# Kkuntal990/video-to-video-diffusion

Measured on AMD Instinct MI355X. Metric: ddim_steps_per_sec, higher is better.
Workload: dtype bf16; 1 GPU; DDIM-50 step (U-Net eval + update) on latent [1, 8, 48, 128, 128] = 8->48 slices @512x512, effective 264.66M U-Net (128x(1,2,4,4), latent 8), one volume per GPU, hipGraph-captured step; volumes_per_gpu=1, parallelism=dp1, full=False, finite_outputs=True

## Files before the change

include/ctsi.h:

```cpp
#ifndef CTSI_H
#define CTSI_H

#include <stddef.h>
#include <stdint.h>

#ifdef __cplusplus
extern "C" {
#endif

#define CTSI_OK 0
#define CTSI_ERR_INVALID (-1)
#define CTSI_ERR_UNSUPPORTED (-2)
#define CTSI_ERR_HIP (-3)

int ctsi_version(void);
int ctsi_ablation_build(void);
const char* ctsi_last_error(void);
int ctsi_device_available(void);

int ctsi_ncdhw_f32_to_ndhwc_bf16(const float* src, void* dst, int n, int c, int d, int h, int w,
                                 int c_total, int c_off, void* stream);
int ctsi_ndhwc_bf16_to_ncdhw_f32(const void* src, float* dst, int n, int c, int d, int h, int w,
                                 void* stream);
int ctsi_ncdhw_f32_to_ndhwc_f32(const float* src, float* dst, int n, int c, int d, int h, int w,
// ... 38 lines not shown
int ctsi_conv_plan_set_stream_tail(ctsi_conv_plan* plan, int on);
void ctsi_conv_plan_destroy(ctsi_conv_plan* plan);
int ctsi_conv_plan_out_dims(const ctsi_conv_plan* plan, int* d_out, int* h_out, int* w_out);
size_t ctsi_conv_plan_weight_bytes(const ctsi_conv_plan* plan);
int ctsi_conv_plan_tiles(const ctsi_conv_plan* plan);
int ctsi_conv_plan_tiles_per_sample(const ctsi_conv_plan* plan);
int ctsi_conv_plan_cout_pad(const ctsi_conv_plan* plan);
size_t ctsi_conv_plan_workspace_bytes(const ctsi_conv_plan* plan);
double ctsi_conv_plan_flops(const ctsi_conv_plan* plan);
int ctsi_conv_plan_config(const ctsi_conv_plan* plan, int* bm, int* bn, int* mode);
int ctsi_conv_plan_form(const ctsi_conv_plan* plan, int out[8]);
#define CTSI_PACK_GATHER 1
#define CTSI_PACK_GATHER_SMALL 2
#define CTSI_PACK_HALO 3
#define CTSI_PACK_K32 4
#define CTSI_PACK_HEAD 5
#define CTSI_PACK_STREAM_TAIL 6
#define CTSI_PACK_STEM 7
int ctsi_conv_plan_pack_layout(const ctsi_conv_plan* plan);
int ctsi_conv_plan_pack_weights(const ctsi_conv_plan* plan, const float* w_f32, void* packed,
                                void* stream);
int ctsi_conv_fwd(const ctsi_conv_plan* plan, const void* x1, const void* x2, const void* packed_w,
                  const float* bias, const ctsi_conv_out* out, void* stream);

int ctsi_gn_colsum(const void* x_bf16, float* colsum, int n, int c, int d, int h, int w,
                   int* tiles_per_sample, void* stream);
int ctsi_gn_colsum_tiles(int d, int h, int w);
int ctsi_gn_finalize(const float* colsum, double* sums, int n, int c, int c_pad, int groups,
                     int tiles_per_sample, int nclass, int accumulate, void* stream);
int ctsi_gn_apply(const void* x_bf16, void* y_bf16, const double* sums, const float* gamma,
                  const float* beta, int n, int c, int d, int h, int w, int d_stat, int groups, float eps,
                  int silu_pre, const float* tbias, int tbias_stride, const int* step_ptr,
                  const void* residual_bf16, int silu_post, void* stream);

int ctsi_attn_pv_supported(int c, int groups);
int ctsi_attn_pv(const float* depthsum, const double* sums, const float* gamma, const float* beta, const void* w_bf16,
                 const float* bias, void* out, int n, int c, int d, int h, int w, int groups, float eps, void* stream);

int ctsi_attn_depthsum(const void* x_bf16, float* depthsum, float* colsum, int n, int c, int d,
                       int h, int w, void* stream);
int ctsi_attn_depthsum_tiles(int c, int h, int w);
int ctsi_attn_normsum(const float* depthsum, const double* sums, const float* gamma,
                      const float* beta, void* out_bf16, int n, int c, int d, int h, int w,
                      int groups, float eps, void* stream);
int ctsi_attn_broadcast_add(const void* x_bf16, const void* p_bf16, const float* rowsum, int heads,
                            void* y_bf16, int n, int c, int d, int h, int w, void* stream);
int ctsi_attn_softmax_rowsum(const void* qk_bf16, float* rowsum, int n, int c, int d, int h, int w,
                             int heads, void* stream);

int ctsi_time_embed_fwd(const int* t_rows, int rows, int dim, int time_dim, const float* w1,
                        const float* b1, const float* w2, const float* b2, const float* w_all,
                        const float* b_all, int total_out, float* scratch, float* tbias_out,
                        void* stream);

int ctsi_time_embed_fwd_tf(const float* t_rows, int rows, int dim, int time_dim, const float* w1,
                           const float* b1, const float* w2, const float* b2, const float* w_all,
                           const float* b_all, int total_out, float* scratch, float* tbias_out,
                           void* stream);

int ctsi_trilinear_depth_fwd(const float* src_f32_ncdhw, void* dst_bf16_ndhwc, int n, int c,
                             int d_in, int d_out, int h, int w, int c_total, int c_off,
                             float* dst_f32_ncdhw, void* stream);

int ctsi_ddim_step(float* z, const float* eps, const float* noise_ncdhw, void* zin_bf16,
                   int c_total, int c_off, const float* coef, const int* step_ptr, int n, int c,
                   int d, int h, int w, int* nonfinite, void* stream);
// ... 174 lines not shown
```

video-to-video-diffusion_amd/csrc/norm_act.hip:

```cpp
#include "ctsi_internal.h"
#include <stdlib.h>

#define GN_TILE_ROWS 512

__device__ __forceinline__ void unpack8(const uint4 v, float* f) {
    f[0] = __uint_as_float(v.x << 16); f[1] = __uint_as_float(v.x & 0xffff0000u);
    f[2] = __uint_as_float(v.y << 16); f[3] = __uint_as_float(v.y & 0xffff0000u);
    f[4] = __uint_as_float(v.z << 16); f[5] = __uint_as_float(v.z & 0xffff0000u);
    f[6] = __uint_as_float(v.w << 16); f[7] = __uint_as_float(v.w & 0xffff0000u);
}
__device__ __forceinline__ uint4 pack8(const float* f) {
    uint4 v;
    v.x = pack_bf16x2(f[0], f[1]); v.y = pack_bf16x2(f[2], f[3]);
    v.z = pack_bf16x2(f[4], f[5]); v.w = pack_bf16x2(f[6], f[7]);
    return v;
}

__global__ void __launch_bounds__(256)
gn_colsum_kernel(const bf16_t* __restrict__ x, float* __restrict__ colsum, int n_total, int c,
                 long long vox_per_sample, int tps) {
    extern __shared__ __attribute__((aligned(16))) char smem_raw[];
    float* s_red = reinterpret_cast<float*>(smem_raw);
    const int cpr = c >> 3;
    const int rows_par = 256 / cpr;
// ... 329 lines not shown
    CTSI_CHECK_ARG(x && y && sums && gamma && beta, "ctsi_gn_apply: null argument");
    CTSI_CHECK_ARG(c % 8 == 0 && groups > 0 && c % groups == 0, "ctsi_gn_apply: bad c=%d groups=%d", c, groups);
    CTSI_CHECK_ARG(d_stat >= d, "ctsi_gn_apply: d_stat=%d < d=%d", d_stat, d);
    const long long vox = (long long)d * h * w;
    const long long total = vox * (c / 8);
    long long blocks = (total + 256 * 8 - 1) / (256 * 8);
    if (blocks > 2048) blocks = 2048;
    if (blocks < 1) blocks = 1;
    const int cpr = c / 8;
    int gq = cpr, g256 = 256;
    while (g256) { const int t = gq % g256; gq = g256; g256 = t; }
    const int need = cpr / gq;
    if (blocks >= need) blocks -= blocks % need;
    bool constq = (blocks * 256) % cpr == 0;
    long long per_block = 0;
    {
        static const char* cg = getenv("CTSI_GN_CONTIG");
        if (!(cg && atoi(cg) == 0) && 256 % cpr == 0) {
            per_block = 1024;
            blocks = (total + per_block - 1) / per_block;
            constq = true;
        }
    }
    const size_t lds = (size_t)c * 3 * sizeof(float);
    static const char* nt_env = getenv("CTSI_GN_NT");
    const bool nt = nt_env ? atoi(nt_env) != 0 : (long long)n * vox * c * 2 > (512ll << 20);
    const int idx = (silu_pre ? 1 : 0) | (tbias ? 2 : 0) | (residual ? 4 : 0) | (silu_post ? 8 : 0) | (constq ? 16 : 0) | (nt ? 32 : 0);
    hipLaunchKernelGGL(gn_apply_pick<0>(idx), dim3((unsigned)blocks, n), dim3(256), lds, (hipStream_t)stream,
                       (const bf16_t*)x, (bf16_t*)y, sums, gamma, beta, c, vox, (long long)d_stat * h * w, groups, eps,
                       tbias, tbias_stride, step_ptr, n, (const bf16_t*)residual, per_block);
    CTSI_LAUNCH_CHECK();
    return CTSI_OK;
}
```

video-to-video-diffusion_amd/engine.py:

```python
from __future__ import annotations

import contextlib
import ctypes as C
import os
import weakref
from typing import Callable, Dict, List, NamedTuple, Optional, Sequence, Tuple

import torch
import torch.nn as nn

from .lib import ConvDesc, ConvOut, CtsiError, get_lib
from .prediction import add_pred_to_eps, check_prediction_type

_CTX: Dict[int, "Ctx"] = {}

_PACKED: Dict[int, "weakref.WeakValueDictionary"] = {}
_LIVE_PROGRAMS: "weakref.WeakSet" = weakref.WeakSet()


def _pack_sig(lib, plan, transposed, k, s, c1: int, c2: int, cout: int, cin_w: Optional[int]) -> tuple:
    bm, bn, mode = C.c_int(), C.c_int(), C.c_int()
    lib.conv_plan_config(plan, C.byref(bm), C.byref(bn), C.byref(mode))
    return (lib.conv_plan_pack_layout(plan), int(transposed), tuple(k), tuple(s), c1, c2, cout, cin_w,
            lib.conv_plan_cout_pad(plan), lib.conv_plan_weight_bytes(plan), bn.value, bm.value,
# ... 631 lines not shown
    def gn_finalize(self, x: Act, groups: int, stats: dict) -> int:
        slot = self._gn_slot(x.n, groups)
        lib, sptr, prog = self.lib, self.ctx.sptr, self
        n, c = x.n, x.c
        parts = stats.get("parts") or [dict(tps=stats["tps"], cpad=stats["cpad"], nclass=stats["nclass"], off=0)]

        def run():
            for i, pt in enumerate(parts):
                lib.gn_finalize(C.c_void_p(prog._colsum.data_ptr() + pt["off"] * 4),
                                C.c_void_p(prog._gn_sums.data_ptr() + slot * 8), n, c, pt["cpad"], groups, pt["tps"],
                                pt["nclass"], int(i > 0), sptr)

        self._emit(run, "gn.finalize", audit=dict(kind="gn_finalize", colsum=lambda: prog._colsum, sums=lambda: prog._gn_sums,
                                                  slot=slot, n=n, c=c, groups=groups, parts=parts))
        return slot

    def gn_colsum(self, x: Act) -> dict:
        lib, sptr, prog = self.lib, self.ctx.sptr, self
        tps = lib.gn_colsum_tiles(x.d, x.h, x.w)
        self._colsum_need = max(self._colsum_need, 2 * x.n * tps * x.c)
        xp = x.ip
        n, c, d, h, w = x.n, x.c, x.d, x.h, x.w

        def run():
            lib.gn_colsum(xp, _ptr(prog._colsum), n, c, d, h, w, None, sptr)

        self._emit(run, "gn.colsum", nbytes=2.0 * n * c * d * h * w,
                   audit=dict(kind="gn_colsum", x=x, colsum=lambda: prog._colsum, tps=tps, tile_rows=512))
        return dict(tps=tps, cpad=x.c, nclass=1)

    def gn_apply(self, x: Act, slot: int, gn: nn.GroupNorm, *, silu_pre: bool, tbias=None,
                 tbias_off: int = 0, tbias_stride: int = 0, step_ptr: Optional[torch.Tensor] = None,
                 residual: Optional[Act] = None, silu_post: bool = False, out: Optional[Act] = None,
                 synced: bool = False) -> Act:
        lib, sptr, prog = self.lib, self.ctx.sptr, self
        if self.shard is not None and not synced:
            self.sync_stats_and_halos(x if x.halo else None, slot, x.n * gn.num_groups * 2)
        if residual is not None and self.shard is not None and residual.halo:
            self.halo_exchange(residual)
        lo, d_ext = self.ext(x)
        gamma = self.dev_f32(lambda: gn.weight)
        beta = self.dev_f32(lambda: gn.bias)
        self.track(gn.weight, gn.bias)
        fresh = out is None
        if out is None:
            out = self.act(x.n, x.c, x.d, x.h, x.w, halo=x.halo)
        out.dirty = bool(self.shard is not None and x.halo and x.dirty)
        xp, yp, gp, bp = self.ext_ptr(x, lo), self.ext_ptr(out, lo), _ptr(gamma), _ptr(beta)
        tbp = C.c_void_p(0 if tbias is None else tbias.data_ptr() + tbias_off * 4)
        stp = _ptr(step_ptr)
        rp = C.c_void_p(0) if residual is None else self.ext_ptr(residual, lo)
        n, c, h, w, groups, eps = x.n, x.c, x.h, x.w, gn.num_groups, float(gn.eps)
        d_stat = self.shard.depth_total if (self.shard is not None and x.halo) else x.d
        d = d_ext

        def run():
            lib.gn_apply(xp, yp, C.c_void_p(prog._gn_sums.data_ptr() + slot * 8), gp, bp, n, c, d, h, w, d_stat,
                         groups, eps, int(silu_pre), tbp, tbias_stride, stp, rp, int(silu_post), sptr)

        self._emit(run, "gn.apply", nbytes=(2 + (residual is not None)) * 2.0 * n * c * d * h * w,
                   audit=dict(kind="gn_apply", x=x, out=out, sums=lambda: prog._gn_sums, slot=slot, gamma=gamma, beta=beta,
                              groups=groups, eps=eps, d_stat=d_stat, silu_pre=bool(silu_pre), tbias=tbias, tbias_off=tbias_off,
                              tbias_stride=tbias_stride, step_ptr=step_ptr, residual=residual, silu_post=bool(silu_post)))
        if fresh:
            self.zero_end_halos(out)
        return out

    def unet_resblock(self, m, x: Act, skip: Optional[Act], tbias: torch.Tensor, tbias_off: int,
                      tbias_stride: int, step_ptr: Optional[torch.Tensor]) -> Act:
        cout = m.conv1.conv.out_channels
        has_res_conv = not isinstance(m.residual_conv, nn.Identity)
        if not has_res_conv and skip is not None:
            raise CtsiError("identity residual with a concatenated input")
        c1, st = self.conv("rb.conv1", lambda: m.conv1.conv.weight, lambda: m.conv1.conv.bias, x, skip,
                           cout=cout, want_stats=True)
        slot = self.gn_finalize(c1, m.conv1.norm.num_groups, st)
        c2, st = self.conv("rb.conv2", lambda: m.conv2[0].weight, lambda: m.conv2[0].bias, c1, None, cout=cout,
                           want_stats=True,
                           norm_in=(slot, m.conv1.norm, True, (tbias, tbias_off, tbias_stride, step_ptr)))
        self.release(c1)
        slot = self.gn_finalize(c2, m.conv2[1].num_groups, st)
        if not has_res_conv:
            return self.gn_apply(c2, slot, m.conv2[1], silu_pre=False, residual=x, silu_post=True, out=c2)
        if os.environ.get("CTSI_NO_FUSE_RES"):
            if self.shard is not None:
                for a in (x, skip):
                    if a is not None:
                        self.halo_exchange(a)
            r, _ = self.conv("res1x1", lambda: m.residual_conv.weight, lambda: m.residual_conv.bias, x, skip,
                             k=(1, 1, 1), p=(0, 0, 0), cout=cout, ext_out=self.shard is not None)
            out = self.gn_apply(c2, slot, m.conv2[1], silu_pre=False, residual=r, silu_post=True, out=c2)
            self.release(r)
            return out
        if self.shard is not None:
            self.sync_stats_and_halos(c2, slot, c2.n * m.conv2[1].num_groups * 2)
            for a in (x, skip):
                if a is not None:
                    self.halo_exchange(a)
        out, _ = self.conv("res1x1+gn", lambda: m.residual_conv.weight, lambda: m.residual_conv.bias, x, skip,
                           k=(1, 1, 1), p=(0, 0, 0), cout=cout, out=c2, fuse_gn=(c2, slot, m.conv2[1], True),
                           ext_out=self.shard is not None)
        return out

    def attention(self, m, x: Act, mode: str = "fast") -> Act:
        lib, sptr, prog = self.lib, self.ctx.sptr, self
        n, c, d, h, w = x.n, x.c, x.d, x.h, x.w
        dev = self.ctx.device
        heads = m.num_heads
        tps = lib.attn_depthsum_tiles(c, h, w)
        self._colsum_need = max(self._colsum_need, 2 * n * tps * c)
        depthsum = self.pool.get(n * h * w * c, torch.float32)
        xp, dsp = x.ip, _ptr(depthsum)
        world = self.shard.world if (self.shard is not None and x.halo) else 1
        d_all = self.shard.depth_total if (self.shard is not None and x.halo) else d

        def run_ds():
            lib.attn_depthsum(xp, dsp, _ptr(prog._colsum), n, c, d, h, w, sptr)

        self._emit(run_ds, "attn.depthsum", nbytes=2.0 * n * c * d * h * w,
                   audit=dict(kind="attn_depthsum", x=x, depthsum=depthsum, colsum=lambda: prog._colsum, tps=tps,
                              tile_pos=256 // (c // 8)))
        slot = self.gn_finalize(x, m.norm.num_groups, dict(tps=tps, cpad=c, nclass=1))
        if self.shard is not None and x.halo:
            self.sync_stats_and_halos(None, slot, n * m.norm.num_groups * 2, f32=depthsum, name="attn.sync")
            self.halo_exchange(x)
        gamma = self.dev_f32(lambda: m.norm.weight)
        beta = self.dev_f32(lambda: m.norm.bias)
        groups, eps = m.norm.num_groups, float(m.norm.eps)
        gp, bp = _ptr(gamma), _ptr(beta)

        def wv():
            return m.qkv.weight[2 * c:3 * c, :, 0, 0, 0].double()

        def wpv():
            wp = m.proj_out.weight[:, :, 0, 0, 0].double()
            return (wp @ wv()).float().reshape(c, c, 1, 1, 1)

        def bpv():
            wp = m.proj_out.weight[:, :, 0, 0, 0].double()
            return (float(d_all) * (wp @ m.qkv.bias[2 * c:3 * c].double()) + m.proj_out.bias.double()).float()

        if lib.attn_pv_supported(c, groups) and not os.environ.get("CTSI_NO_ATTN_PV"):
            wbuf = self.persistent((c, c), torch.bfloat16)
            self.pack_fns.append(lambda: wbuf.copy_(wpv().reshape(c, c).to(device=dev, dtype=torch.bfloat16)))
            bias_pv = self.dev_f32(bpv)
            pterm = self.act(n, c, 1, h, w, halo=0)
            wp_, bpp, ptp = _ptr(wbuf), _ptr(bias_pv), _ptr(pterm.t)

            def run_pv():
                lib.attn_pv(dsp, C.c_void_p(prog._gn_sums.data_ptr() + slot * 8), gp, bp, wp_, bpp, ptp, n, c, d_all, h, w,
                            groups, eps, sptr)

            fl_pv = 2.0 * n * h * w * c * c
            self.flops += fl_pv
# ... 113 lines not shown
                self.lib.graph_destroy(self._fast["graph"])
        except Exception:
            pass


class SamplerStep(NamedTuple):
    entry: str
    noise: bool
    hist: bool
    nonfinite: bool


SAMPLER_STEPS = {
    "ddim": SamplerStep("ddim_step", noise=True, hist=False, nonfinite=True),
    "ddpm": SamplerStep("ddpm_step", noise=True, hist=False, nonfinite=False),
    "dpmpp": SamplerStep("dpm_step", noise=False, hist=True, nonfinite=True),
    "heun": SamplerStep("heun_step", noise=True, hist=True, nonfinite=True),
}


def sampler_step_launcher(lib, kind: str, f32: bool) -> Callable:
    s = SAMPLER_STEPS[kind]
    fn = getattr(lib, s.entry + ("_f32" if f32 else ""))

    def launch(z, eps, hist, noise, zin, c_total, coef, step_ptr, n, L, d, h, w, nonfinite, stream):
        ops = [z, eps] + ([hist] if s.hist else []) + ([noise] if s.noise else [])
        tail = [nonfinite] if s.nonfinite else []
        fn(*ops, zin, c_total, 0, coef, step_ptr, n, L, d, h, w, *tail, stream)
    return launch


class UNetProgram(Program):

    def __init__(self, ctx: Ctx, unet, n: int, d: int, h: int, w: int, max_rows: int, attention_mode="fast",
                 shard=None, guided: bool = False, rescale: bool = False, prediction: str = "epsilon"):
        super().__init__(ctx)
        self.shard = shard
        if shard is not None and n != 1:
            raise CtsiError("depth-sharded programs support one volume per rank")
        if shard is not None and guided:
            raise CtsiError("classifier-free guidance does not support depth sharding: the sharded program holds one "
                            "volume per rank and the rescale statistics would need a collective")
        self.unet = unet
        self.guided, self.rescale = bool(guided), bool(guided and rescale)
        self.prediction = check_prediction_type(prediction)
        self.n, self.d, self.h, self.w = n, d, h, w
        n = self.nb = 2 * n if guided else n
        L = unet.latent_dim
        self.L = L
        dev = ctx.device
        self.attention_mode = attention_mode
        self.max_rows = max_rows
        halo = 0 if shard is None else 1
        self.xin, self.xin2 = self._input_acts(n, d, h, w, halo)
        self.eps = self.persistent((n, d, h, w, L), torch.float32)
        self.z = self.persistent((self.n, d, h, w, L), torch.float32, zero=True)
        self.step_ptr = self.persistent((1,), torch.int32, zero=True)
        self.t_rows = self.persistent((max_rows,), torch.int32, zero=True)
        self.t_rows_f = self.persistent((max_rows,), torch.float32, zero=True)
        self.coef = self.persistent((max_rows, 8), torch.float32, zero=True)
        self.noise = None
        self.track_module(unet)

        te = unet.time_embed.time_mlp
        self.dim = unet.model_channels
        self.time_dim = te[1].out_features
        blocks = [m for m in unet.modules() if type(m).__name__ == "ResBlock3D"]
        self.tb_off = {}
        off = 0
        for m in blocks:
            self.tb_off[id(m)] = off
            off += m.time_mlp[1].out_features
        self.total_out = off
        self.w1 = self.dev_f32(lambda: te[1].weight)
        self.b1 = self.dev_f32(lambda: te[1].bias)
        self.w2 = self.dev_f32(lambda: te[3].weight)
        self.b2 = self.dev_f32(lambda: te[3].bias)
        self.w_all = self.dev_f32(lambda: torch.cat([m.time_mlp[1].weight for m in blocks], 0))
        self.b_all = self.dev_f32(lambda: torch.cat([m.time_mlp[1].bias for m in blocks], 0))
        self.tbias = self.persistent((max_rows, self.total_out), torch.float32, zero=True)
        self.te_scratch = self.persistent((max_rows * (self.dim + 2 * self.time_dim),), torch.float32)

        self.zero_gn_op()
        x, _ = self.conv("conv_in", lambda: unet.conv_in.weight, lambda: unet.conv_in.bias, self.xin, self.xin2,
                         cout=unet.conv_in.out_channels)
        skips: List[Act] = []

        def step(layer, xcur: Act, skip: Optional[Act] = None) -> Act:
            ynew = self._layer(layer, xcur, skip)
            if not any(xcur is sk for sk in skips):
                self.release(xcur)
            if skip is not None:
                self.release(skip)
            return ynew

        for level_blocks, down in zip(unet.down_blocks, unet.down_samples):
            for block_list in level_blocks:
                for layer in block_list:
                    x = step(layer, x)
            skips.append(x)
            if not isinstance(down, nn.Identity):
                x, _ = self.conv("down", (lambda m=down: m.conv.weight), (lambda m=down: m.conv.bias), x, None,
                                 k=(3, 4, 4), s=(2, 2), p=(1, 1, 1), cout=down.conv.out_channels)
        x = step(unet.mid_block1, x)
        x = step(unet.mid_attn, x)
        x = step(unet.mid_block2, x)
        for level_blocks, up in zip(unet.up_blocks, unet.up_samples):
            for j, block_list in enumerate(level_blocks):
                skip = skips.pop() if j == 0 else None
                for layer in block_list:
                    x = step(layer, x, skip)
                    skip = None
            if not isinstance(up, nn.Identity):
                xo, _ = self.conv("up", (lambda m=up: m.conv.weight), (lambda m=up: m.conv.bias), x, None,
                                  transposed=True, k=(3, 4, 4), s=(2, 2), p=(1, 1, 1),
                                  cout=up.conv.out_channels)
                self.release(x)
                x = xo
        gn, conv = unet.conv_out[0], unet.conv_out[2]
        st = self.gn_colsum(x)
        slot = self.gn_finalize(x, gn.num_groups, st)
        y = self.gn_apply(x, slot, gn, silu_pre=True)
        self.release(x)
        vox = d * h * w
        self.conv("conv_out", lambda: conv.weight, lambda: conv.bias, y, None, cout=L, f32_out=self.eps,
                  f32_strides=(vox * L, 1, h * w * L, w * L, L))
        self.release(y)
        self.unet_op_count = len(self.ops)
        self.finalize_layout()

    def _input_acts(self, n, d, h, w, halo) -> Tuple[Act, Optional[Act]]:
        L = self.L
        return Act(self.persistent((n * (d + 2 * halo) * h * w * 2 * L,), torch.bfloat16, zero=True), n, 2 * L, d, h, w,
                   halo), None

    def _layer(self, layer, x: Act, skip: Optional[Act]) -> Act:
        kind = type(layer).__name__
        if kind == "ResBlock3D":
            return self.unet_resblock(layer, x, skip, self.tbias, self.tb_off[id(layer)], self.total_out,
                                      self.step_ptr)
        if kind == "TemporalAttention":
            return self.attention(layer, x, self.attention_mode)
        raise CtsiError(f"unsupported U-Net layer {kind}")

    def load_latents(self, z_ncdhw: Optional[torch.Tensor], cond_ncdhw: Optional[torch.Tensor]):
        lib, sptr = self.lib, self.ctx.sptr
        n, L, d, h, w = self.n, self.L, self.d, self.h, self.w
        lo = 0 if self.shard is None else self.shard.depth_start
        if z_ncdhw is not None:
            z = z_ncdhw.detach()[:, :, lo:lo + d].to(device=self.ctx.device, dtype=torch.float32).contiguous()
            lib.ncdhw_f32_to_ndhwc_f32(_ptr(z), _ptr(self.z), n, L, d, h, w, sptr)
            lib.ncdhw_f32_to_ndhwc_bf16(_ptr(z), self.xin.ip, n, L, d, h, w, 2 * L, 0, sptr)
            if self.guided:
                lib.ncdhw_f32_to_ndhwc_bf16(_ptr(z), self._uncond_zin(), n, L, d, h, w, 2 * L, 0, sptr)
            z.record_stream(self.ctx.stream)
            self.xin.dirty = True
        if cond_ncdhw is not None:
            cnd = cond_ncdhw.detach()[:, :, lo:lo + d].to(device=self.ctx.device, dtype=torch.float32).contiguous()
            lib.ncdhw_f32_to_ndhwc_bf16(_ptr(cnd), self.xin.ip, n, L, d, h, w, 2 * L, L, sptr)
            cnd.record_stream(self.ctx.stream)

    def set_guidance(self, scale: float, rescale: float = 0.0):
        if not self.guided:
            raise CtsiError("internal: set_guidance on a program built without guidance")
        if rescale > 0.0 and not self.rescale:
            raise CtsiError("internal: guidance_rescale > 0 needs a program built with the statistics pass")
        row = torch.tensor([float(scale), float(rescale)], dtype=torch.float32)
        self.cfg_scale.copy_(row.expand(self.cfg_scale.shape[0], 2))

    def set_schedule(self, t_rows: Sequence[float], coef_rows: Optional[torch.Tensor] = None,
                     pred_rows: Optional[torch.Tensor] = None):
        rows = len(t_rows)
        if rows > self.max_rows:
            raise CtsiError(f"schedule needs {rows} rows but the program was built for {self.max_rows}")
        lib, sptr = self.lib, self.ctx.sptr
# ... 312 lines not shown
```

video-to-video-diffusion_amd/engine_f32.py:

```python
from __future__ import annotations

import ctypes as C
import weakref
from typing import List, Optional, Tuple

import torch
import torch.nn as nn

from .engine import (_PACKED, Act, Ctx, UNetProgram, VAEDecodeProgram, VAEEncodeProgram, _content_key,
                     _ptr)
from .lib import ConvDesc, ConvOut, CtsiError

PRECISIONS = ("bf16", "fp32")


def _f32_pack_sig(desc: ConvDesc, cout_pad: int, wbytes: int) -> tuple:
    return ("fp32", int(desc.transposed), (desc.kd, desc.kh, desc.kw), (desc.sh, desc.sw), desc.c1, desc.c2, desc.cout,
            cout_pad, wbytes)


def check_precision(p) -> str:
    if not isinstance(p, str) or p not in PRECISIONS:
        raise ValueError(f"unknown inference precision {p!r}: expected one of {PRECISIONS}")
    return p


class _F32Ops:

    precision = "fp32"

    def act(self, n, c, d, h, w, halo: Optional[int] = None) -> Act:
        if halo:
            raise CtsiError("the fp32 inference mode does not support depth sharding")
        return Act(self.pool.get(n * c * d * h * w, torch.float32), n, c, d, h, w, 0)

    def conv(self, name: str, weight_fn, bias_fn, x1: Act, x2: Optional[Act], *, transposed=False, k=(3, 3, 3), s=(1, 1),
             p=(1, 1, 1), cout: int, cin_w: Optional[int] = None, out: Optional[Act] = None, want_stats=False,
             f32_out: Optional[torch.Tensor] = None, f32_strides=None, act: int = 0, fuse_gn=None, ext_out: bool = False,
             norm_in=None, residual: Optional[Act] = None):
        lib, prog = self.lib, self
        if fuse_gn is not None or ext_out:
            raise CtsiError("internal: the fused GroupNorm tail / halo-extended outputs are bf16-path features")
        c2 = 0 if x2 is None else x2.c
        if cin_w is not None and cin_w != x1.c + c2:
            raise CtsiError(f"internal: fp32 activations carry no padding channels (cin_w={cin_w}, c={x1.c + c2})")
        if x2 is not None and (x2.n, x2.d, x2.h, x2.w) != (x1.n, x1.d, x1.h, x1.w):
            raise CtsiError("internal: concatenated sources of different shapes")
        if norm_in is not None:
            nslot, ngn, nsilu, ntb = norm_in
            kw_tb = {} if ntb is None else dict(tbias=ntb[0], tbias_off=ntb[1], tbias_stride=ntb[2], step_ptr=ntb[3])
            self.gn_apply(x1, nslot, ngn, silu_pre=nsilu, out=x1, **kw_tb)
        desc = ConvDesc(int(transposed), k[0], k[1], k[2], s[0], s[1], p[0], p[1], p[2], x1.n, x1.c, c2, cout, x1.d, x1.h,
                        x1.w, 0)
        if not lib.conv_f32_supported(C.byref(desc)):
            raise CtsiError(f"{name}: {lib.last_error().decode()}")
        self.keep.append(desc)
        do, ho, wo, tps, ncls, cpad = (C.c_int() for _ in range(6))
        lib.conv_f32_geometry(C.byref(desc), C.byref(do), C.byref(ho), C.byref(wo), C.byref(tps), C.byref(ncls),
                              C.byref(cpad))
        do, ho, wo, tps, ncls, cpad = do.value, ho.value, wo.value, tps.value, ncls.value, cpad.value
# ... 241 lines not shown
```

video-to-video-diffusion_amd/lib.py:

```python
from __future__ import annotations

import ctypes as C
import os
import subprocess
from pathlib import Path

_PKG_DIR = Path(__file__).resolve().parent
LIB_PATH = _PKG_DIR / "libctsi.so"
CSRC_DIR = _PKG_DIR / "csrc"
HEADER_PATH = _PKG_DIR.parent / "include" / "ctsi.h"


class CtsiError(RuntimeError):
    """Raised when libctsi is unavailable or one of its entry points reports an error."""


class ConvDesc(C.Structure):
    _fields_ = [
        ("transposed", C.c_int),
        ("kd", C.c_int), ("kh", C.c_int), ("kw", C.c_int),
        ("sh", C.c_int), ("sw", C.c_int),
        ("pd", C.c_int), ("ph", C.c_int), ("pw", C.c_int),
        ("n", C.c_int), ("c1", C.c_int), ("c2", C.c_int),
        ("cout", C.c_int),
# ... 34 lines not shown
_vp, _i, _f, _ll, _sz = C.c_void_p, C.c_int, C.c_float, C.c_longlong, C.c_size_t
_ip = C.POINTER(C.c_int)

SIGNATURES = {
    "ctsi_version": (_i, [], False),
    "ctsi_ablation_build": (_i, [], False),
    "ctsi_last_error": (C.c_char_p, [], False),
    "ctsi_device_available": (_i, [], False),
    "ctsi_ncdhw_f32_to_ndhwc_bf16": (_i, [_vp, _vp, _i, _i, _i, _i, _i, _i, _i, _vp], True),
    "ctsi_ndhwc_bf16_to_ncdhw_f32": (_i, [_vp, _vp, _i, _i, _i, _i, _i, _vp], True),
    "ctsi_ncdhw_f32_to_ndhwc_f32": (_i, [_vp, _vp, _i, _i, _i, _i, _i, _vp], True),
    "ctsi_ndhwc_f32_to_ncdhw_f32": (_i, [_vp, _vp, _i, _i, _i, _i, _i, _vp], True),
    "ctsi_conv_plan_create": (_i, [C.POINTER(_vp), C.POINTER(ConvDesc)], True),
    "ctsi_conv_plan_set_weight_cin": (_i, [_vp, _i], True),
    "ctsi_conv_plan_set_stream_tail": (_i, [_vp, _i], True),
    "ctsi_conv_plan_destroy": (None, [_vp], False),
    "ctsi_conv_plan_out_dims": (_i, [_vp, _ip, _ip, _ip], True),
    "ctsi_conv_plan_weight_bytes": (_sz, [_vp], False),
    "ctsi_conv_plan_workspace_bytes": (_sz, [_vp], False),
    "ctsi_conv_plan_tiles": (_i, [_vp], False),
    "ctsi_conv_plan_tiles_per_sample": (_i, [_vp], False),
    "ctsi_conv_plan_cout_pad": (_i, [_vp], False),
    "ctsi_conv_plan_flops": (C.c_double, [_vp], False),
    "ctsi_conv_plan_config": (_i, [_vp, _ip, _ip, _ip], True),
    "ctsi_conv_plan_pack_layout": (_i, [_vp], False),
    "ctsi_conv_plan_form": (_i, [_vp, _ip], True),
    "ctsi_conv_plan_pack_weights": (_i, [_vp, _vp, _vp, _vp], True),
    "ctsi_conv_fwd": (_i, [_vp, _vp, _vp, _vp, _vp, C.POINTER(ConvOut), _vp], True),
    "ctsi_gn_colsum": (_i, [_vp, _vp, _i, _i, _i, _i, _i, _ip, _vp], True),
    "ctsi_gn_colsum_tiles": (_i, [_i, _i, _i], False),
    "ctsi_gn_finalize": (_i, [_vp, _vp, _i, _i, _i, _i, _i, _i, _i, _vp], True),
    "ctsi_gn_apply": (_i, [_vp, _vp, _vp, _vp, _vp, _i, _i, _i, _i, _i, _i, _i, _f, _i, _vp, _i, _vp, _vp,
                           _i, _vp], True),
    "ctsi_attn_depthsum": (_i, [_vp, _vp, _vp, _i, _i, _i, _i, _i, _vp], True),
    "ctsi_attn_depthsum_tiles": (_i, [_i, _i, _i], False),
    "ctsi_attn_normsum": (_i, [_vp, _vp, _vp, _vp, _vp, _i, _i, _i, _i, _i, _i, _f, _vp], True),
    "ctsi_attn_pv_supported": (_i, [_i, _i], False),
    "ctsi_attn_pv": (_i, [_vp, _vp, _vp, _vp, _vp, _vp, _vp, _i, _i, _i, _i, _i, _i, _f, _vp], True),
    "ctsi_attn_broadcast_add": (_i, [_vp, _vp, _vp, _i, _vp, _i, _i, _i, _i, _i, _vp], True),
    "ctsi_attn_softmax_rowsum": (_i, [_vp, _vp, _i, _i, _i, _i, _i, _i, _vp], True),
    "ctsi_time_embed_fwd": (_i, [_vp, _i, _i, _i, _vp, _vp, _vp, _vp, _vp, _vp, _i, _vp, _vp, _vp], True),
    "ctsi_time_embed_fwd_tf": (_i, [_vp, _i, _i, _i, _vp, _vp, _vp, _vp, _vp, _vp, _i, _vp, _vp, _vp], True),
    "ctsi_trilinear_depth_fwd": (_i, [_vp, _vp, _i, _i, _i, _i, _i, _i, _i, _i, _vp, _vp], True),
    "ctsi_ddim_step": (_i, [_vp, _vp, _vp, _vp, _i, _i, _vp, _vp, _i, _i, _i, _i, _i, _vp, _vp], True),
    "ctsi_ddpm_step": (_i, [_vp, _vp, _vp, _vp, _i, _i, _vp, _vp, _i, _i, _i, _i, _i, _vp], True),
    "ctsi_ddpm_posterior": (_i, [_vp, _vp, _vp, _vp, _vp, _vp, _i, _ll, _i, _vp], True),
    "ctsi_step_advance": (_i, [_vp, _vp], True),
    "ctsi_nan_to_num_f32": (_i, [_vp, _ll, _vp], True),
    "ctsi_count_nonfinite_f32": (_i, [_vp, _ll, _i, _vp, _vp], True),
    "ctsi_wgrad_workspace_bytes": (_sz, [C.POINTER(WgradDesc)], False),
    "ctsi_wgrad_flops": (C.c_double, [C.POINTER(WgradDesc)], False),
    "ctsi_wgrad": (_i, [C.POINTER(WgradDesc), _vp, _vp, _vp, _sz, _vp, _ll, _ll, _ll, _f, _vp], True),
    "ctsi_weight_dgrad_layout": (_i, [_vp, _vp, _i, _i, _i, _i, _i, _vp], True),
    "ctsi_linear_wgrad_multi": (_i, [_vp, _vp, _i, _vp], True),
    "ctsi_gn_bwd_tiles": (_i, [_i, _i, _i], False),
    "ctsi_gn_bwd_workspace_floats": (_sz, [_i, _i, _i, _i, _i, _i], False),
    "ctsi_gn_bwd": (_i, [_vp, _vp, _i, _vp, _vp, _vp, _i, _i, _i, _i, _i, _i, _f, _i, _vp, _i, _vp, _vp, _vp, _vp,
                         _vp, _vp, _vp, _ll, _vp, _vp], True),
    "ctsi_channel_sum_workspace_floats": (_sz, [_ll, _i], False),
    "ctsi_channel_sum": (_i, [_vp, _ll, _i, _i, _vp, _vp, _f, _vp], True),
    "ctsi_add_bf16": (_i, [_vp, _vp, _ll, _vp], True),
    "ctsi_f32_to_bf16": (_i, [_vp, _vp, _ll, _vp], True),
    "ctsi_vae_head_grad": (_i, [_vp, _vp, _i, _i, _i, _i, _i, _f, _i, _vp, _i, _vp], True),
    "ctsi_thin_wgrad_workspace_bytes": (_sz, [_i, _i, _i, _i, _i], False),
    "ctsi_thin_wgrad_supported": (_i, [_i, _i, _i, _i, _i], False),
    "ctsi_thin_wgrad": (_i, [_vp, _i, _i, _vp, _i, _i, _i, _i, _i, _i, _i, _i, _i, _vp, _sz, _vp, _f, _vp], True),
# ... 126 lines not shown
```

Before: 40.18 steps/s.

## Fuse GroupNorm statistics of next layer into resblock GN-apply tail

Adds GN-apply kernels for the silu(gn(x)+residual) resblock tail that also emit the next layer's statistics: column sums for the final output GroupNorm, and depth sums plus column sums for a following temporal attention. The engine tracks the layer sequence and hands these precomputed statistics forward, so the separate colsum and depthsum passes are skipped. This removes one full bf16 read of the activation per fused site. In exchange the fused kernels do extra reductions and LDS traffic, and the launch grid for colsum (one block per 512-row tile, using only rows_par lanes) may be less efficient than the original apply kernel. The path is single-GPU only and falls back for large tensors over 512 MiB.

```diff
diff --git a/include/ctsi.h b/include/ctsi.h
--- a/include/ctsi.h
+++ b/include/ctsi.h
@@ -94,6 +94,15 @@
                   const float* beta, int n, int c, int d, int h, int w, int d_stat, int groups, float eps,
                   int silu_pre, const float* tbias, int tbias_stride, const int* step_ptr,
                   const void* residual_bf16, int silu_post, void* stream);
+int ctsi_gn_apply_colsum(const void* x_bf16, void* y_bf16, const double* sums, const float* gamma,
+                         const float* beta, int n, int c, int d, int h, int w, int d_stat, int groups, float eps,
+                         int silu_pre, const float* tbias, int tbias_stride, const int* step_ptr,
+                         const void* residual_bf16, int silu_post, float* colsum, void* stream);
+int ctsi_gn_apply_depthsum(const void* x_bf16, void* y_bf16, const double* sums, const float* gamma,
+                           const float* beta, int n, int c, int d, int h, int w, int d_stat, int groups, float eps,
+                           int silu_pre, const float* tbias, int tbias_stride, const int* step_ptr,
+                           const void* residual_bf16, int silu_post, float* depthsum, float* colsum, void* stream);
+int ctsi_gn_apply_fused_ok(int kind, int n, int c, int d, int h, int w);
 
 int ctsi_attn_pv_supported(int c, int groups);
 int ctsi_attn_pv(const float* depthsum, const double* sums, const float* gamma, const float* beta, const void* w_bf16,
diff --git a/video-to-video-diffusion_amd/csrc/norm_act.hip b/video-to-video-diffusion_amd/csrc/norm_act.hip
--- a/video-to-video-diffusion_amd/csrc/norm_act.hip
+++ b/video-to-video-diffusion_amd/csrc/norm_act.hip
@@ -385,3 +385,283 @@
     CTSI_LAUNCH_CHECK();
     return CTSI_OK;
 }
+
+__device__ __forceinline__ void gn_coefs_to_lds(float* s_scale, float* s_shift, const double* __restrict__ sums,
+                                                const float* __restrict__ gamma, const float* __restrict__ beta, int nb, int c,
+                                                int groups, long long vox_stat, float eps) {
+    const int cpg = c / groups;
+    const double cnt = (double)cpg * (double)vox_stat;
+    for (int ch = threadIdx.x; ch < c; ch += 256) {
+        const int g = ch / cpg;
+        const double m = sums[((long long)nb * groups + g) * 2 + 0] / cnt;
+        double var = sums[((long long)nb * groups + g) * 2 + 1] / cnt - m * m;
+        if (var < 0.0) var = 0.0;
+        const float rstd = (float)(1.0 / sqrt(var + (double)eps));
+        const float sc = gamma[ch] * rstd;
+        s_scale[ch] = sc;
+        s_shift[ch] = beta[ch] - (float)m * sc;
+    }
+}
+
+__device__ __forceinline__ uint4 gn_tail8(const uint4 raw, const uint4 rraw, const float* sc, const float* sh, float* f) {
+    const uint32_t xin[4] = {raw.x, raw.y, raw.z, raw.w}, rin[4] = {rraw.x, rraw.y, rraw.z, rraw.w};
+    uint32_t o[4];
+#pragma unroll
+    for (int j = 0; j < 4; ++j) {
+        f32x2_t v = {__uint_as_float(xin[j] << 16), __uint_as_float(xin[j] & 0xffff0000u)};
+        const f32x2_t s2 = {sc[2 * j], sc[2 * j + 1]}, h2 = {sh[2 * j], sh[2 * j + 1]};
+        v = v * s2 + h2;
+        v += f32x2_t{__uint_as_float(rin[j] << 16), __uint_as_float(rin[j] & 0xffff0000u)};
+        v = silu2_f(v);
+        o[j] = pack_bf16x2_v(v);
+    }
+    const uint4 packed = make_uint4(o[0], o[1], o[2], o[3]);
+    unpack8(packed, f);
+    return packed;
+}
+
+__global__ void __launch_bounds__(256)
+gn_apply_colsum_kernel(const bf16_t* x, bf16_t* y, const double* __restrict__ sums, const float* __restrict__ gamma,
+                       const float* __restrict__ beta, int c, long long vox, long long vox_stat, int groups, float eps,
+                       const bf16_t* __restrict__ residual, float* __restrict__ colsum, int n_total, int tps) {
+    extern __shared__ __attribute__((aligned(16))) char smem_raw[];
+    float* s_scale = reinterpret_cast<float*>(smem_raw);
+    float* s_shift = s_scale + c;
+    float* s_red = s_shift + c;
+    const int cpr = c >> 3;
+    const int rows_par = 256 / cpr;
+    const int tid = threadIdx.x;
+    const int q = tid % cpr, rl = tid / cpr;
+    const int tile = blockIdx.x, nb = blockIdx.y;
+    gn_coefs_to_lds(s_scale, s_shift, sums, gamma, beta, nb, c, groups, vox_stat, eps);
+    __syncthreads();
+    const long long v0 = (long long)tile * GN_TILE_ROWS;
+    long long v1 = v0 + GN_TILE_ROWS;
+    if (v1 > vox) v1 = vox;
+    float s1[8], s2[8];
+#pragma unroll
+    for (int k = 0; k < 8; ++k) s1[k] = s2[k] = 0.0f;
+    if (rl < rows_par) {
+        float sc[8], sh[8];
+#pragma unroll
+        for (int k = 0; k < 8; ++k) {
+            sc[k] = s_scale[q * 8 + k];
+            sh[k] = s_shift[q * 8 + k];
+        }
+        const long long off = ((long long)nb * vox) * c + q * 8;
+        const bf16_t* xb = x + off;
+        const bf16_t* rb = residual + off;
+        bf16_t* yb = y + off;
+        constexpr int U = 4;
+        long long v = v0 + rl;
+        auto tally = [&](const uint4 raw, const uint4 rraw, long long vv) {
+            float f[8];
+            *reinterpret_cast<uint4*>(yb + vv * c) = gn_tail8(raw, rraw, sc, sh, f);
+#pragma unroll
+            for (int k = 0; k < 8; ++k) {
+                s1[k] += f[k];
+                s2[k] += f[k] * f[k];
+            }
+        };
+        for (; v + (U - 1) * rows_par < v1; v += U * rows_par) {
+            uint4 raw[U], rraw[U];
+#pragma unroll
+            for (int u = 0; u < U; ++u) {
+                raw[u] = *reinterpret_cast<const uint4*>(xb + (v + u * rows_par) * c);
+                rraw[u] = *reinterpret_cast<const uint4*>(rb + (v + u * rows_par) * c);
+            }
+#pragma unroll
+            for (int u = 0; u < U; ++u) tally(raw[u], rraw[u], v + u * rows_par);
+        }
+        for (; v < v1; v += rows_par)
+            tally(*reinterpret_cast<const uint4*>(xb + v * c), *reinterpret_cast<const uint4*>(rb + v * c), v);
+#pragma unroll
+        for (int k = 0; k < 8; ++k) {
+            s_red[((rl * c) + q * 8 + k) * 2 + 0] = s1[k];
+            s_red[((rl * c) + q * 8 + k) * 2 + 1] = s2[k];
+        }
+    }
+    __syncthreads();
+    for (int col = tid; col < c; col += 256) {
+        float t1 = 0.0f, t2 = 0.0f;
+        for (int r = 0; r < rows_par; ++r) {
+            t1 += s_red[(r * c + col) * 2 + 0];
+            t2 += s_red[(r * c + col) * 2 + 1];
+        }
+        const long long tg = (long long)nb * tps + tile;
+        const long long slab = (long long)n_total * tps * c;
+        colsum[tg * c + col] = t1;
+        colsum[slab + tg * c + col] = t2;
+    }
+}
+
+template <int U>
+__global__ void __launch_bounds__(256)
+gn_apply_depthsum_kernel(const bf16_t* x, bf16_t* y, const double* __restrict__ sums, const float* __restrict__ gamma,
+                         const float* __restrict__ beta, int c, int d, int hw, long long vox_stat, int groups, float eps,
+                         const bf16_t* __restrict__ residual, float* __restrict__ depthsum, float* __restrict__ colsum,
+                         int n_total, int tps) {
+    extern __shared__ __attribute__((aligned(16))) char smem_raw[];
+    float* s_scale = reinterpret_cast<float*>(smem_raw);
+    float* s_shift = s_scale + c;
+    float* s_red = s_shift + c;
+    const int cpr = c >> 3;
+    const int rows_par = 256 / cpr;
+    const int tid = threadIdx.x;
+    const int q = tid % cpr, rl = tid / cpr;
+    const int tile = blockIdx.x, nb = blockIdx.y;
+    gn_coefs_to_lds(s_scale, s_shift, sums, gamma, beta, nb, c, groups, vox_stat, eps);
+    __syncthreads();
+    float c1[8], c2[8];
+#pragma unroll
+    for (int k = 0; k < 8; ++k) c1[k] = c2[k] = 0.0f;
+    if (rl < rows_par) {
+        const int pos = tile * rows_par + rl;
+        if (pos < hw) {
+            float sc[8], sh[8];
+#pragma unroll
+            for (int k = 0; k < 8; ++k) {
+                sc[k] = s_scale[q * 8 + k];
+                sh[k] = s_shift[q * 8 + k];
+            }
+            float s[8];
+#pragma unroll
+            for (int k = 0; k < 8; ++k) s[k] = 0.0f;
+            const long long off = (((long long)nb * d) * hw + pos) * c + q * 8;
+            const bf16_t* xb = x + off;
+            const bf16_t* rb = residual + off;
+            bf16_t* yb = y + off;
+            const long long dstride = (long long)hw * c;
+            int dd = 0;
+            for (; dd + U <= d; dd += U) {
+                uint4 raw[U], rraw[U];
+#pragma unroll
+                for (int u = 0; u < U; ++u) {
+                    raw[u] = *reinterpret_cast<const uint4*>(xb + (dd + u) * dstride);
+                    rraw[u] = *reinterpret_cast<const uint4*>(rb + (dd + u) * dstride);
+                }
+#pragma unroll
+                for (int u = 0; u < U; ++u) {
+                    float f[8];
+                    *reinterpret_cast<uint4*>(yb + (dd + u) * dstride) = gn_tail8(raw[u], rraw[u], sc, sh, f);
+#pragma unroll
+                    for (int k = 0; k < 8; ++k) {
+                        s[k] += f[k];
+                        c2[k] += f[k] * f[k];
+                    }
+                }
+            }
+            for (; dd < d; ++dd) {
+                const uint4 raw = *reinterpret_cast<const uint4*>(xb + dd * dstride);
+                const uint4 rraw = *reinterpret_cast<const uint4*>(rb + dd * dstride);
+                float f[8];
+                *reinterpret_cast<uint4*>(yb + dd * dstride) = gn_tail8(raw, rraw, sc, sh, f);
+#pragma unroll
+                for (int k = 0; k < 8; ++k) {
+                    s[k] += f[k];
+                    c2[k] += f[k] * f[k];
+                }
+            }
+            float* o = depthsum + ((long long)nb * hw + pos) * c + q * 8;
+            *reinterpret_cast<float4*>(o) = make_float4(s[0], s[1], s[2], s[3]);
+            *reinterpret_cast<float4*>(o + 4) = make_float4(s[4], s[5], s[6], s[7]);
+#pragma unroll
+            for (int k = 0; k < 8; ++k) c1[k] += s[k];
+        }
+#pragma unroll
+        for (int k = 0; k < 8; ++k) {
+            s_red[(rl * c + q * 8 + k) * 2 + 0] = c1[k];
+            s_red[(rl * c + q * 8 + k) * 2 + 1] = c2[k];
+        }
+    }
+    __syncthreads();
+    for (int col = tid; col < c; col += 256) {
+        float t1 = 0.0f, t2 = 0.0f;
+        for (int r = 0; r < rows_par; ++r) {
+            t1 += s_red[(r * c + col) * 2 + 0];
+            t2 += s_red[(r * c + col) * 2 + 1];
+        }
+        const long long tg = (long long)nb * tps + tile;
+        const long long slab = (long long)n_total * tps * c;
+        colsum[tg * c + col] = t1;
+        colsum[slab + tg * c + col] = t2;
+    }
+}
+
+extern "C" int ctsi_gn_apply_fused_ok(int kind, int n, int c, int d, int h, int w) {
+    if (kind != 0 && kind != 1) return 0;
+    if (n < 1 || d < 1 || h < 1 || w < 1 || c < 8 || c % 8 != 0 || c > 2048) return 0;
+    static const char* force = getenv("CTSI_FUSE_STATS_FORCE");
+    if (force) return atoi(force) != 0;
+    if ((long long)n * d * h * w * c * 2 > (512ll << 20)) return 0;
+    if (kind == 1) {
+        const int rows_par = 256 / (c / 8);
+        if (ctsi_attn_depthsum_tiles(c, h, w) != (h * w + rows_par - 1) / rows_par) return 0;
+    }
+    return 1;
+}
+
+static int gn_apply_fused_args(const char* who, const void* x, const void* y, const double* sums, const float* gamma,
+                               const float* beta, int c, int d, int d_stat, int groups, int silu_pre, const float* tbias,
+                               const void* residual, int silu_post) {
+    if (!(x && y && sums && gamma && beta)) {
+        ctsi_set_error("%s: null argument", who);
+        return CTSI_ERR_INVALID;
+    }
+    if (!(c % 8 == 0 && c >= 8 && c <= 2048 && groups > 0 && c % groups == 0)) {
+        ctsi_set_error("%s: bad c=%d groups=%d (c a multiple of 8 in [8,2048])", who, c, groups);
+        return CTSI_ERR_INVALID;
+    }
+    if (d_stat < d) {
+        ctsi_set_error("%s: d_stat=%d < d=%d", who, d_stat, d);
+        return CTSI_ERR_INVALID;
+    }
+    if (silu_pre || tbias || !residual || !silu_post) {
+        ctsi_set_error("%s: only the identity-residual tail silu(gn(x) + residual) is instantiated "
+                       "(silu_pre=%d tbias=%d residual=%d silu_post=%d)", who, silu_pre, tbias != nullptr, residual != nullptr,
+                       silu_post);
+        return CTSI_ERR_UNSUPPORTED;
+    }
+    return CTSI_OK;
+}
+
+extern "C" int ctsi_gn_apply_colsum(const void* x, void* y, const double* sums, const float* gamma, const float* beta,
+                                    int n, int c, int d, int h, int w, int d_stat, int groups, float eps, int silu_pre,
+                                    const float* tbias, int tbias_stride, const int* step_ptr, const void* residual,
+                                    int silu_post, float* colsum, void* stream) {
+    const int rc = gn_apply_fused_args("ctsi_gn_apply_colsum", x, y, sums, gamma, beta, c, d, d_stat, groups, silu_pre, tbias,
+                                       residual, silu_post);
+    if (rc != CTSI_OK) return rc;
+    CTSI_CHECK_ARG(colsum, "ctsi_gn_apply_colsum: null colsum");
+    const int tps = ctsi_gn_colsum_tiles(d, h, w);
+    const int rows_par = 256 / (c / 8);
+    const size_t lds = ((size_t)2 * c + (size_t)rows_par * c * 2) * sizeof(float);
+    hipLaunchKernelGGL(gn_apply_colsum_kernel, dim3(tps, n), dim3(256), lds, (hipStream_t)stream, (const bf16_t*)x, (bf16_t*)y,
+                       sums, gamma, beta, c, (long long)d * h * w, (long long)d_stat * h * w, groups, eps,
+                       (const bf16_t*)residual, colsum, n, tps);
+    CTSI_LAUNCH_CHECK();
+    return CTSI_OK;
+}
+
+extern "C" int ctsi_gn_apply_depthsum(const void* x, void* y, const double* sums, const float* gamma, const float* beta,
+                                      int n, int c, int d, int h, int w, int d_stat, int groups, float eps, int silu_pre,
+                                      const float* tbias, int tbias_stride, const int* step_ptr, const void* residual,
+                                      int silu_post, float* depthsum, float* colsum, void* stream) {
+    const int rc = gn_apply_fused_args("ctsi_gn_apply_depthsum", x, y, sums, gamma, beta, c, d, d_stat, groups, silu_pre, tbias,
+                                       residual, silu_post);
+    if (rc != CTSI_OK) return rc;
+    CTSI_CHECK_ARG(depthsum && colsum, "ctsi_gn_apply_depthsum: null depthsum / colsum");
+    const int tps = ctsi_attn_depthsum_tiles(c, h, w);
+    const int rows_par = 256 / (c / 8);
+    if (tps != (h * w + rows_par - 1) / rows_par) {
+        ctsi_set_error("ctsi_gn_apply_depthsum: ctsi_attn_depthsum walks more than one round of positions per block");
+        return CTSI_ERR_UNSUPPORTED;
+    }
+    const size_t lds = ((size_t)2 * c + (size_t)rows_par * c * 2) * sizeof(float);
+    auto kern = (long long)tps * n <= 256 ? gn_apply_depthsum_kernel<8> : gn_apply_depthsum_kernel<4>;
+    hipLaunchKernelGGL(kern, dim3(tps, n), dim3(256), lds, (hipStream_t)stream, (const bf16_t*)x,
+                       (bf16_t*)y, sums, gamma, beta, c, d, h * w, (long long)d_stat * h * w, groups, eps,
+                       (const bf16_t*)residual, depthsum, colsum, n, tps);
+    CTSI_LAUNCH_CHECK();
+    return CTSI_OK;
+}
diff --git a/video-to-video-diffusion_amd/engine.py b/video-to-video-diffusion_amd/engine.py
--- a/video-to-video-diffusion_amd/engine.py
+++ b/video-to-video-diffusion_amd/engine.py
@@ -687,8 +687,11 @@
     def gn_apply(self, x: Act, slot: int, gn: nn.GroupNorm, *, silu_pre: bool, tbias=None,
                  tbias_off: int = 0, tbias_stride: int = 0, step_ptr: Optional[torch.Tensor] = None,
                  residual: Optional[Act] = None, silu_post: bool = False, out: Optional[Act] = None,
-                 synced: bool = False) -> Act:
+                 synced: bool = False, emit: Optional[str] = None):
         lib, sptr, prog = self.lib, self.ctx.sptr, self
+        if emit is not None and (emit not in ("colsum", "depthsum") or self.shard is not None or residual is None
+                                 or not silu_post or silu_pre or tbias is not None):
+            raise CtsiError(f"gn_apply(emit={emit!r}): only the identity-residual tail of a single-GPU program emits statistics")
         if self.shard is not None and not synced:
             self.sync_stats_and_halos(x if x.halo else None, slot, x.n * gn.num_groups * 2)
         if residual is not None and self.shard is not None and residual.halo:
@@ -708,21 +711,44 @@
         n, c, h, w, groups, eps = x.n, x.c, x.h, x.w, gn.num_groups, float(gn.eps)
         d_stat = self.shard.depth_total if (self.shard is not None and x.halo) else x.d
         d = d_ext
+        stats, extra, depthsum = None, 0.0, None
+        if emit == "colsum":
+            stats = dict(tps=lib.gn_colsum_tiles(d, h, w), cpad=c, nclass=1)
+        elif emit == "depthsum":
+            depthsum = self.pool.get(n * h * w * c, torch.float32)
+            stats = dict(tps=lib.attn_depthsum_tiles(c, h, w), cpad=c, nclass=1, depthsum=depthsum)
+            extra = 4.0 * n * h * w * c
+        if stats is not None:
+            self._colsum_need = max(self._colsum_need, 2 * n * stats["tps"] * c)
+            extra += 4.0 * 2 * n * stats["tps"] * c
+        dsp = _ptr(depthsum)
 
         def run():
-            lib.gn_apply(xp, yp, C.c_void_p(prog._gn_sums.data_ptr() + slot * 8), gp, bp, n, c, d, h, w, d_stat,
-                         groups, eps, int(silu_pre), tbp, tbias_stride, stp, rp, int(silu_post), sptr)
-
-        self._emit(run, "gn.apply", nbytes=(2 + (residual is not None)) * 2.0 * n * c * d * h * w,
+            args = (xp, yp, C.c_void_p(prog._gn_sums.data_ptr() + slot * 8), gp, bp, n, c, d, h, w, d_stat,
+                    groups, eps, int(silu_pre), tbp, tbias_stride, stp, rp, int(silu_post))
+            if emit is None:
+                lib.gn_apply(*args, sptr)
+            elif emit == "colsum":
+                lib.gn_apply_colsum(*args, _ptr(prog._colsum), sptr)
+            else:
+                lib.gn_apply_depthsum(*args, dsp, _ptr(prog._colsum), sptr)
+
+        self._emit(run, "gn.apply", nbytes=(2 + (residual is not None)) * 2.0 * n * c * d * h * w + extra,
                    audit=dict(kind="gn_apply", x=x, out=out, sums=lambda: prog._gn_sums, slot=slot, gamma=gamma, beta=beta,
                               groups=groups, eps=eps, d_stat=d_stat, silu_pre=bool(silu_pre), tbias=tbias, tbias_off=tbias_off,
-                              tbias_stride=tbias_stride, step_ptr=step_ptr, residual=residual, silu_post=bool(silu_post)))
+                              tbias_stride=tbias_stride, step_ptr=step_ptr, residual=residual, silu_post=bool(silu_post),
+                              emit=emit))
         if fresh:
             self.zero_end_halos(out)
-        return out
+        return out if emit is None else (out, stats)
+
+    def _emitted_stats_fresh(self, x: Act, emit: str):
+        rec = self.op_audit[-1] if self.op_audit else None
+        if not (rec is not None and rec.get("kind") == "gn_apply" and rec.get("emit") == emit and rec["out"] is x):
+            raise CtsiError(f"statistics emitted by a ResBlock tail ({emit}) must be finalised by the very next op")
 
     def unet_resblock(self, m, x: Act, skip: Optional[Act], tbias: torch.Tensor, tbias_off: int,
-                      tbias_stride: int, step_ptr: Optional[torch.Tensor]) -> Act:
+                      tbias_stride: int, step_ptr: Optional[torch.Tensor], emit: Optional[str] = None):
         cout = m.conv1.conv.out_channels
         has_res_conv = not isinstance(m.residual_conv, nn.Identity)
         if not has_res_conv and skip is not None:
@@ -736,7 +762,17 @@
         self.release(c1)
         slot = self.gn_finalize(c2, m.conv2[1].num_groups, st)
         if not has_res_conv:
-            return self.gn_apply(c2, slot, m.conv2[1], silu_pre=False, residual=x, silu_post=True, out=c2)
+            kind = {"colsum": 0, "depthsum": 1}.get(emit)
+            if (kind is not None and self.shard is None
+                    and (kind == 0 or self.lib.attn_depthsum_tiles(c2.c, c2.h, c2.w) > 0)
+                    and self.lib.gn_apply_fused_ok(kind, c2.n, c2.c, c2.d, c2.h, c2.w)):
+                return self.gn_apply(c2, slot, m.conv2[1], silu_pre=False, residual=x, silu_post=True, out=c2, emit=emit)
+            out = self.gn_apply(c2, slot, m.conv2[1], silu_pre=False, residual=x, silu_post=True, out=c2)
+            return out if emit is None else (out, None)
+        out = self._unet_resblock_conv_tail(m, x, skip, c2, slot, cout)
+        return out if emit is None else (out, None)
+
+    def _unet_resblock_conv_tail(self, m, x: Act, skip: Optional[Act], c2: Act, slot: int, cout: int) -> Act:
         if os.environ.get("CTSI_NO_FUSE_RES"):
             if self.shard is not None:
                 for a in (x, skip):
@@ -757,24 +793,31 @@
                            ext_out=self.shard is not None)
         return out
 
-    def attention(self, m, x: Act, mode: str = "fast") -> Act:
+    def attention(self, m, x: Act, mode: str = "fast", pre: Optional[dict] = None) -> Act:
         lib, sptr, prog = self.lib, self.ctx.sptr, self
         n, c, d, h, w = x.n, x.c, x.d, x.h, x.w
         dev = self.ctx.device
         heads = m.num_heads
         tps = lib.attn_depthsum_tiles(c, h, w)
-        self._colsum_need = max(self._colsum_need, 2 * n * tps * c)
-        depthsum = self.pool.get(n * h * w * c, torch.float32)
-        xp, dsp = x.ip, _ptr(depthsum)
         world = self.shard.world if (self.shard is not None and x.halo) else 1
         d_all = self.shard.depth_total if (self.shard is not None and x.halo) else d
-
-        def run_ds():
-            lib.attn_depthsum(xp, dsp, _ptr(prog._colsum), n, c, d, h, w, sptr)
-
-        self._emit(run_ds, "attn.depthsum", nbytes=2.0 * n * c * d * h * w,
-                   audit=dict(kind="attn_depthsum", x=x, depthsum=depthsum, colsum=lambda: prog._colsum, tps=tps,
-                              tile_pos=256 // (c // 8)))
+        if pre is not None:
+            self._emitted_stats_fresh(x, "depthsum")
+            depthsum = pre["depthsum"]
+            if pre["tps"] != tps or depthsum.numel() < n * h * w * c:
+                raise CtsiError("attention: the precomputed statistics do not fit this tensor")
+            dsp = _ptr(depthsum)
+        else:
+            self._colsum_need = max(self._colsum_need, 2 * n * tps * c)
+            depthsum = self.pool.get(n * h * w * c, torch.float32)
+            xp, dsp = x.ip, _ptr(depthsum)
+
+            def run_ds():
+                lib.attn_depthsum(xp, dsp, _ptr(prog._colsum), n, c, d, h, w, sptr)
+
+            self._emit(run_ds, "attn.depthsum", nbytes=2.0 * n * c * d * h * w,
+                       audit=dict(kind="attn_depthsum", x=x, depthsum=depthsum, colsum=lambda: prog._colsum, tps=tps,
+                                  tile_pos=256 // (c // 8)))
         slot = self.gn_finalize(x, m.norm.num_groups, dict(tps=tps, cpad=c, nclass=1))
         if self.shard is not None and x.halo:
             self.sync_stats_and_halos(None, slot, n * m.norm.num_groups * 2, f32=depthsum, name="attn.sync")
@@ -954,10 +997,14 @@
 
 class UNetProgram(Program):
 
+    FUSE_STATS = True
+
     def __init__(self, ctx: Ctx, unet, n: int, d: int, h: int, w: int, max_rows: int, attention_mode="fast",
                  shard=None, guided: bool = False, rescale: bool = False, prediction: str = "epsilon"):
         super().__init__(ctx)
         self.shard = shard
+        self.fuse_stats = bool(self.FUSE_STATS and shard is None and not guided
+                               and os.environ.get("CTSI_NO_FUSE_STATS", "0") in ("", "0"))
         if shard is not None and n != 1:
             raise CtsiError("depth-sharded programs support one volume per rank")
         if shard is not None and guided:
@@ -1007,9 +1054,27 @@
         x, _ = self.conv("conv_in", lambda: unet.conv_in.weight, lambda: unet.conv_in.bias, self.xin, self.xin2,
                          cout=unet.conv_in.out_channels)
         skips: List[Act] = []
+        seq: List[object] = []
+        for level_blocks, down in zip(unet.down_blocks, unet.down_samples):
+            seq += [layer for block_list in level_blocks for layer in block_list]
+            seq += [] if isinstance(down, nn.Identity) else ["down"]
+        seq += [unet.mid_block1, unet.mid_attn, unet.mid_block2]
+        for level_blocks, up in zip(unet.up_blocks, unet.up_samples):
+            seq += [layer for block_list in level_blocks for layer in block_list]
+            seq += [] if isinstance(up, nn.Identity) else ["up"]
+        seq.append("out")
+        self._stats_pre: Optional[dict] = None
+        pos = [0]
 
         def step(layer, xcur: Act, skip: Optional[Act] = None) -> Act:
-            ynew = self._layer(layer, xcur, skip)
+            while seq[pos[0]] is not layer:
+                pos[0] += 1
+            nxt = seq[pos[0] + 1]
+            pos[0] += 1
+            emit = None
+            if self.fuse_stats and type(layer).__name__ == "ResBlock3D":
+                emit = "depthsum" if type(nxt).__name__ == "TemporalAttention" else "colsum" if nxt == "out" else None
+            ynew = self._layer(layer, xcur, skip, emit)
             if not any(xcur is sk for sk in skips):
                 self.release(xcur)
             if skip is not None:
@@ -1040,7 +1105,11 @@
                 self.release(x)
                 x = xo
         gn, conv = unet.conv_out[0], unet.conv_out[2]
-        st = self.gn_colsum(x)
+        st, self._stats_pre = self._stats_pre, None
+        if st is not None:
+            self._emitted_stats_fresh(x, "colsum")
+        else:
+            st = self.gn_colsum(x)
         slot = self.gn_finalize(x, gn.num_groups, st)
         y = self.gn_apply(x, slot, gn, silu_pre=True)
         self.release(x)
@@ -1056,13 +1125,20 @@
         return Act(self.persistent((n * (d + 2 * halo) * h * w * 2 * L,), torch.bfloat16, zero=True), n, 2 * L, d, h, w,
                    halo), None
 
-    def _layer(self, layer, x: Act, skip: Optional[Act]) -> Act:
+    def _layer(self, layer, x: Act, skip: Optional[Act], emit: Optional[str] = None) -> Act:
         kind = type(layer).__name__
+        pre, self._stats_pre = self._stats_pre, None
         if kind == "ResBlock3D":
-            return self.unet_resblock(layer, x, skip, self.tbias, self.tb_off[id(layer)], self.total_out,
-                                      self.step_ptr)
+            if emit is None:
+                return self.unet_resblock(layer, x, skip, self.tbias, self.tb_off[id(layer)], self.total_out,
+                                          self.step_ptr)
+            out, self._stats_pre = self.unet_resblock(layer, x, skip, self.tbias, self.tb_off[id(layer)], self.total_out,
+                                                      self.step_ptr, emit=emit)
+            return out
         if kind == "TemporalAttention":
-            return self.attention(layer, x, self.attention_mode)
+            if pre is None:
+                return self.attention(layer, x, self.attention_mode)
+            return self.attention(layer, x, self.attention_mode, pre=pre)
         raise CtsiError(f"unsupported U-Net layer {kind}")
 
     def load_latents(self, z_ncdhw: Optional[torch.Tensor], cond_ncdhw: Optional[torch.Tensor]):
diff --git a/video-to-video-diffusion_amd/engine_f32.py b/video-to-video-diffusion_amd/engine_f32.py
--- a/video-to-video-diffusion_amd/engine_f32.py
+++ b/video-to-video-diffusion_amd/engine_f32.py
@@ -26,6 +26,8 @@
 
 
 class _F32Ops:
+
+    FUSE_STATS = False
 
     precision = "fp32"
 
diff --git a/video-to-video-diffusion_amd/lib.py b/video-to-video-diffusion_amd/lib.py
--- a/video-to-video-diffusion_amd/lib.py
+++ b/video-to-video-diffusion_amd/lib.py
@@ -90,6 +90,11 @@
     "ctsi_gn_finalize": (_i, [_vp, _vp, _i, _i, _i, _i, _i, _i, _i, _vp], True),
     "ctsi_gn_apply": (_i, [_vp, _vp, _vp, _vp, _vp, _i, _i, _i, _i, _i, _i, _i, _f, _i, _vp, _i, _vp, _vp,
                            _i, _vp], True),
+    "ctsi_gn_apply_colsum": (_i, [_vp, _vp, _vp, _vp, _vp, _i, _i, _i, _i, _i, _i, _i, _f, _i, _vp, _i, _vp, _vp,
+                                  _i, _vp, _vp], True),
+    "ctsi_gn_apply_depthsum": (_i, [_vp, _vp, _vp, _vp, _vp, _i, _i, _i, _i, _i, _i, _i, _f, _i, _vp, _i, _vp, _vp,
+                                    _i, _vp, _vp, _vp], True),
+    "ctsi_gn_apply_fused_ok": (_i, [_i, _i, _i, _i, _i, _i], False),
     "ctsi_attn_depthsum": (_i, [_vp, _vp, _vp, _i, _i, _i, _i, _i, _vp], True),
     "ctsi_attn_depthsum_tiles": (_i, [_i, _i, _i], False),
     "ctsi_attn_normsum": (_i, [_vp, _vp, _vp, _vp, _vp, _i, _i, _i, _i, _i, _i, _f, _vp], True),
```

Result: no change. 40.31 steps/s, median of 6 (+0.3%).
